# hpcaitech/Open-Sora

Hardware: AMD Instinct MI355X
Metric: latent_frames_per_sec (30-step rectified-flow sampling; denoise-step ms in ms_per_step) (higher is better)
Workload: dtype bf16; 1 GPU; MMDiT-XL (hidden 1152, 16x72, 9+19 blocks) denoise step, latent 16x64x64 (16x512x512 px), L=16896 tokens, CFG batch 3, 30-step Euler sampling; cfg_batch=3, parallelism=single GPU

## Files before the change

### open_sora_amd/csrc/gemm256x.hip

```cpp
#include "acc_quads.h"
#include "gemm_epilogue16.h"
#include "tile256.h"
#include "gemm256x_regs.inc"

namespace osk_gemm {
namespace {

struct GeoX {
  static constexpr int NB = OSKX_NB;
  template <int T>
  OSK_DEV void read(const osk_v4f* aq, float* v4) {
#pragma unroll
    for (int i = 0; i < 4; ++i) asm volatile("v_accvgpr_read_b32 %0, %1" : "=v"(v4[i]) : "a"(aq[T][i]));
  }
};

template <int NP>
struct GemmPack {
  GemmParams p[NP];
};

#ifdef OSK_GEMM_TILE_TIMING
__device__ unsigned long long osk_gemm_tile_ticks[4];
#define OSK_TT(i, t0) if (threadIdx.x == 0) atomicAdd(&osk_gemm_tile_ticks[i], __builtin_amdgcn_s_memtime() - (t0))
#else
#define OSK_TT(i, t0)
#endif


template <bool OUT_F32>
struct LinearWalk {
  template <int NP>
  OSK_DEV int col_tiles(const GemmPack<NP>& pk, int) { return (pk.p[0].N - pk.p[0].skip_len + 255) / 256; }
  template <int NP>
  OSK_DEV int phys_n0(const GemmPack<NP>& pk, int n0) { return n0 + (n0 >= pk.p[0].skip_from ? pk.p[0].skip_len : 0); }
  OSK_DEV int64_t a_row(const GemmParams& p, int m) { return osk_tile256::a_row_offset(p, m); }
  OSK_DEV int64_t w_row(const GemmParams& p, int n, bool) { return osk_tile256::w_row_offset(p, n); }
  OSK_DEV bool affine(const GemmParams& p, int m0, int n0) {
    return m0 + 256 <= p.M && n0 + 256 <= p.N && m0 / p.arpb == (m0 + 255) / p.arpb;
  }
  OSK_DEV int64_t a_origin(const GemmParams& p, int m0) { return osk_tile256::tile_window(m0, p.M, p.arpb, 0x7fffffff, p.abs_, p.ars).lo; }
  OSK_DEV int64_t w_origin(const GemmParams& p, int n0) { return osk_tile256::tile_window(n0, p.N, 0x7fffffff, 0x7fffffff, 0, p.wrs).lo; }
  OSK_DEV bool folded(const GemmParams& p, int n0w) { return p.bias != nullptr && n0w + OSKX_NB * 16 <= p.N; }
  OSK_DEV void epilogue(const osk_v4f* aq, const GemmParams& p, int m0w, int n0w, int l15, int q4, bool folded) {
    constexpr int WT = OSKX_NB * 16;
    const int b_first = m0w / p.crpb, b_last = (m0w + WT - 1) / p.crpb;
    const bool interior = m0w + WT <= p.M && n0w + WT <= p.N && b_first == b_last;
    epi16::epilogue_all<GeoX, OUT_F32>(aq, p, m0w, n0w, l15, q4, interior, folded);
  }
};

struct VtWalk {
  template <int NP>
  OSK_DEV int col_tiles(const GemmPack<NP>& pk, int i) { return (pk.p[i].N + 255) / 256; }
  template <int NP>
  OSK_DEV int phys_n0(const GemmPack<NP>&, int n0) { return n0; }
  OSK_DEV int64_t a_row(const GemmParams& p, int m) {
    m = m < p.M ? m : p.M - 1;
    return (int64_t)m * p.ars;
  }
  OSK_DEV int64_t w_row(const GemmParams& p, int n, bool permute) {
    n = n < p.N ? n : p.N - 1;
    const int wb = n / p.wrpb;
    int pos = n - wb * p.wrpb;
    if (permute) pos = vt_perm64(pos, p.vt);
    pos = pos < p.wvalid ? pos : p.wvalid - 1;
    return wb * p.wbs + (int64_t)pos * p.wrs;
  }
  OSK_DEV bool affine(const GemmParams& p, int m0, int n0) {
    const int wb = n0 / p.wrpb, pos0 = n0 - wb * p.wrpb;
    return m0 + 256 <= p.M && n0 + 256 <= p.N && pos0 + 256 <= p.wrpb && pos0 + 256 <= p.wvalid;
  }
  OSK_DEV int64_t a_origin(const GemmParams& p, int m0) { return osk_tile256::tile_window(m0, p.M, 0x7fffffff, 0x7fffffff, 0, p.ars).lo; }
  OSK_DEV int64_t w_origin(const GemmParams& p, int n0) { return osk_tile256::tile_window(n0, p.N, p.wrpb, p.wvalid, p.wbs, p.wrs).lo; }
  OSK_DEV bool folded(const GemmParams&, int) { return false; }
  OSK_DEV void epilogue(const osk_v4f* aq, const GemmParams& p, int m0w, int n0w, int l15, int q4, bool) {
    epi16::vt_all<GeoX>(aq, p, m0w, n0w, l15, q4);
  }
};

#define OSKW_OPERANDS                                                                                               \
  ::"v"(faA0), "v"(faW0), "v"(aoff[0]), "v"(aoff[1]), "v"(aoff[2]), "v"(aoff[3]), "v"(aoff[4]), "v"(aoff[5]),          \
      "v"(aoff[6]), "v"(aoff[7]), "v"(woff[0]), "v"(woff[1]), "v"(woff[2]), "v"(woff[3]), "v"(woff[4]), "v"(woff[5]),  \
      "v"(woff[6]), "v"(woff[7]), "v"(boff), "s"(abase), "s"(wbase), "s"(bbase), "s"(nk), "s"(adst), "s"(wdst),        \
      "s"(flags), "s"(abasen), "s"(wbasen), "v"(aoffp), "v"(woffp)

template <class Walk, int NP>
OSK_DEV void tile_walk(const GemmPack<NP>& pk) {
  constexpr int WT = OSKX_NB * 16;
  extern __shared__ __attribute__((aligned(16))) unsigned char smem[];
  const int tid = threadIdx.x;
  const int lane = tid & 63;
  const int wave = __builtin_amdgcn_readfirstlane(tid >> 6);
  const int wm = wave >> 1, wn = wave & 1;
  const int q4 = lane >> 4, l15 = lane & 15;

  const int nbn0 = Walk::col_tiles(pk, 0), nbn1 = Walk::col_tiles(pk, NP - 1);
  const int nt0 = ((pk.p[0].M + 255) / 256) * nbn0;
  const int ntiles = NP == 1 ? nt0 : nt0 + ((pk.p[NP - 1].M + 255) / 256) * nbn1;
  const int grp = pk.p[0].group > 0 ? pk.p[0].group : 1;
  auto tile_of = [&](int it, int& sel, int& m0, int& n0) {
    int tile = xcd_remap(it, ntiles);
    sel = (NP > 1 && tile >= nt0) ? 1 : 0;
    tile -= sel ? nt0 : 0;
    const osk_tile256::TileBlock t = osk_tile256::grouped_tile(tile, (pk.p[sel].M + 255) / 256, sel ? nbn1 : nbn0, grp);
    m0 = t.bm * 256;
    n0 = Walk::phys_n0(pk, t.bn * 256);
  };
  const unsigned lds_base = (unsigned)(uintptr_t)(__attribute__((address_space(3))) unsigned char*)smem;
  const unsigned sz0 = (unsigned)((q4 ^ ((l15 >> 1) & 7)) << 4);
  const unsigned faA0 = lds_base + (wm * WT + l15) * 128 + sz0;
  const unsigned faW0 = lds_base + OSKX_W_BASE + (wn * WT + l15) * 128 + sz0;
  const unsigned nk = rfl((unsigned)(pk.p[0].K / 64));
  const unsigned adst = rfl(lds_base + wave * 1024), wdst = rfl(lds_base + OSKX_W_BASE + wave * 1024);

  unsigned prefetched = 0;
  for (int it = blockIdx.x; it < ntiles; it += (int)gridDim.x) {
    const int itn = it + (int)gridDim.x;
#ifdef OSK_GEMM_TILE_TIMING
    const unsigned long long tt0 = __builtin_amdgcn_s_memtime();
#endif
    int sel, m0, n0, seln = 0, m0n = 0, n0n = 0;
    tile_of(it, sel, m0, n0);
    const GemmParams& p = pk.p[NP == 1 ? 0 : sel];
    bool has_next = itn < ntiles;
    const int64_t alo = Walk::a_origin(p, m0), wlo = Walk::w_origin(p, n0);
    int64_t alon = alo, wlon = wlo;
    if (has_next) {
      tile_of(itn, seln, m0n, n0n);
      has_next = seln == sel && Walk::affine(p, m0, n0) && Walk::affine(p, m0n, n0n);
      alon = Walk::a_origin(p, m0n);
      wlon = Walk::w_origin(p, n0n);
    }
    const uint64_t abase = rfl64((uint64_t)(uintptr_t)p.A + (uint64_t)(alo * 2)), wbase = rfl64((uint64_t)(uintptr_t)p.W + (uint64_t)(wlo * 2));
    const uint64_t abasen = rfl64((uint64_t)(uintptr_t)p.A + (uint64_t)(alon * 2)), wbasen = rfl64((uint64_t)(uintptr_t)p.W + (uint64_t)(wlon * 2));
    const uint64_t bbase = rfl64((uint64_t)(uintptr_t)p.bias);
    unsigned aoff[8], woff[8];
#pragma unroll
    for (int i = 0; i < 8; ++i) {
      const int r = osk_tile256::dma_row<4>(wave, lane, i);
      const int c = osk_tile256::dma_chunk(lane, r);
      aoff[i] = (unsigned)((Walk::a_row(p, m0 + r) - alo) * 2 + c * 16);
      woff[i] = (unsigned)((Walk::w_row(p, n0 + r, true) - wlo) * 2 + c * 16);
    }
    const int m0w = m0 + wm * WT, n0w = n0 + wn * WT;
    const bool folded = Walk::folded(p, n0w);
    const unsigned boff = (unsigned)((n0w + q4 * 4) * 4);
    const unsigned flags = rfl(prefetched | (has_next ? 2u : 0u) | (folded ? 4u : 0u));
    const unsigned aoffp = (unsigned)((Walk::a_row(p, m0 + wave * 64 + lane) - alo) * 2);
    const unsigned woffp = (unsigned)((Walk::w_row(p, n0 + wave * 64 + lane, false) - wlo) * 2);
    OSK_TT(0, tt0);
#ifdef OSK_GEMM_TILE_TIMING
    const unsigned long long tt1 = __builtin_amdgcn_s_memtime();
#endif
    asm volatile(
#include "gemm256x_body.inc"
        OSKW_OPERANDS : OSKX_CLOBBERS);
    static_assert(OSKX_ACC_QUADS == 64, "the generated loop's accumulator map: quad T = tile T, a0 .. a255");
    osk_v4f aq[64];
    asm volatile("" : OSK_AQ_OUT_0_64(aq));
    OSK_TT(1, tt1);
#ifdef OSK_GEMM_TILE_TIMING
    const unsigned long long tt2 = __builtin_amdgcn_s_memtime();
#endif
    Walk::epilogue(aq, p, m0w, n0w, l15, q4, folded);
    OSK_TT(2, tt2);
#ifdef OSK_GEMM_TILE_TIMING
    if (threadIdx.x == 0) atomicAdd(&osk_gemm_tile_ticks[3], 1ull);
#endif
    prefetched = has_next ? 1u : 0u;
  }
}

#undef OSKW_OPERANDS

template <bool OUT_F32, int NP>
__global__ void __launch_bounds__(256, 1) gemm256x_kernel(const GemmPack<NP> pk) {
  tile_walk<LinearWalk<OUT_F32>>(pk);
}

template <int NP>
__global__ void __launch_bounds__(256, 1) gemm256x_vt_kernel(const GemmPack<NP> pk) {
  static_assert(NP <= 2, "a run-time index into a wider pack makes hipcc copy the pack to scratch");
  tile_walk<VtWalk>(pk);
}

int tiles_of(const GemmParams& p) { return ((p.M + 255) / 256) * ((p.N - p.skip_len + 255) / 256); }

template <bool OUT_F32>
int launch_one(const GemmParams& p, hipStream_t st) {
  auto kernel = gemm256x_kernel<OUT_F32, 1>;
  OSK_ENSURE_MAX_SMEM(kernel, OSKX_SMEM);
  GemmPack<1> pk;
  pk.p[0] = p;
  hipLaunchKernelGGL(kernel, dim3(osk_tile256::persistent_grid(tiles_of(p))), dim3(256), OSKX_SMEM, st, pk);
  return (int)hipGetLastError();
}

}

#ifdef OSK_GEMM_TILE_TIMING
extern "C" int osk_gemm_tile_timing_read(unsigned long long* out4) {
  unsigned long long zero[4] = {0, 0, 0, 0};
  if (hipMemcpyFromSymbol(out4, HIP_SYMBOL(osk_gemm_tile_ticks), sizeof(zero)) != hipSuccess) return -1;
  return hipMemcpyToSymbol(HIP_SYMBOL(osk_gemm_tile_ticks), zero, sizeof(zero)) == hipSuccess ? 0 : -1;
}
#endif

int launch_gemm256x(const GemmParams& p, int out_f32, hipStream_t st) {
  return out_f32 ? launch_one<true>(p, st) : launch_one<false>(p, st);
}

int launch_gemm256x_pair(const GemmParams& p0, const GemmParams& p1, hipStream_t st) {
  auto kernel = gemm256x_kernel<false, 2>;
  OSK_ENSURE_MAX_SMEM(kernel, OSKX_SMEM);
  GemmPack<2> pk;
  pk.p[0] = p0;
  pk.p[1] = p1;
  hipLaunchKernelGGL(kernel, dim3(osk_tile256::persistent_grid(tiles_of(p0) + tiles_of(p1))), dim3(256), OSKX_SMEM, st, pk);
  return (int)hipGetLastError();
}

int launch_gemm256x_vt(const GemmParams* ps, int n, hipStream_t st) {
  if (n < 1 || n > 2) return OSK_EINVAL;
  auto kernel = gemm256x_vt_kernel<2>;
  OSK_ENSURE_MAX_SMEM(kernel, OSKX_SMEM);
  GemmPack<2> pk;
  int ntiles = 0;
  for (int i = 0; i < 2; ++i) {
    pk.p[i] = ps[i < n ? i : 0];
    if (i >= n) pk.p[i].M = 0;
    ntiles += tiles_of(pk.p[i]);
  }
  hipLaunchKernelGGL(kernel, dim3(osk_tile256::persistent_grid(ntiles)), dim3(256), OSKX_SMEM, st, pk);
  return (int)hipGetLastError();
}

}
```

### open_sora_amd/csrc/gemm256x_body.inc

```
"  s_mov_b64 s[40:41], %19\n"
"  s_mov_b64 s[42:43], %20\n"
"  s_mov_b64 s[54:55], %21\n"
"  s_mov_b32 s44, %22\n"
"  s_mov_b32 s45, %23\n"
"  s_mov_b32 s46, %24\n"
"  s_mov_b32 s52, %25\n"
"  s_mov_b32 s47, 0\n"
"  s_mov_b32 s48, 0\n"
"  v_xor_b32_e32 v224, 64, %0\n"
"  v_xor_b32_e32 v225, 64, %1\n"
"  s_bitcmp1_b32 s52, 0\n"
"  s_cbranch_scc1 .Lx256_have0_%=\n"
"  s_add_u32 m0, s45, 0\n"
"  s_nop 0\n"
"  global_load_lds_dwordx4 %2, s[40:41]\n"
"  s_add_u32 m0, s45, 4096\n"
"  s_nop 0\n"
"  global_load_lds_dwordx4 %3, s[40:41]\n"
"  s_add_u32 m0, s45, 8192\n"
"  s_nop 0\n"
"  global_load_lds_dwordx4 %4, s[40:41]\n"
"  s_add_u32 m0, s45, 12288\n"
"  s_nop 0\n"
"  global_load_lds_dwordx4 %5, s[40:41]\n"
"  s_add_u32 m0, s45, 16384\n"
"  s_nop 0\n"
"  global_load_lds_dwordx4 %6, s[40:41]\n"
"  s_add_u32 m0, s45, 20480\n"
"  s_nop 0\n"
"  global_load_lds_dwordx4 %7, s[40:41]\n"
"  s_add_u32 m0, s45, 24576\n"
"  s_nop 0\n"
"  global_load_lds_dwordx4 %8, s[40:41]\n"
"  s_add_u32 m0, s45, 28672\n"
"  s_nop 0\n"
"  global_load_lds_dwordx4 %9, s[40:41]\n"
"  s_add_u32 m0, s46, 0\n"
"  s_nop 0\n"
"  global_load_lds_dwordx4 %10, s[42:43]\n"
"  s_add_u32 m0, s46, 4096\n"
"  s_nop 0\n"
"  global_load_lds_dwordx4 %11, s[42:43]\n"
"  s_add_u32 m0, s46, 8192\n"
"  s_nop 0\n"
"  global_load_lds_dwordx4 %12, s[42:43]\n"
"  s_add_u32 m0, s46, 12288\n"
"  s_nop 0\n"
"  global_load_lds_dwordx4 %13, s[42:43]\n"
"  s_add_u32 m0, s46, 16384\n"
"  s_nop 0\n"
"  global_load_lds_dwordx4 %14, s[42:43]\n"
"  s_add_u32 m0, s46, 20480\n"
"  s_nop 0\n"
"  global_load_lds_dwordx4 %15, s[42:43]\n"
"  s_add_u32 m0, s46, 24576\n"
"  s_nop 0\n"
"  global_load_lds_dwordx4 %16, s[42:43]\n"
"  s_add_u32 m0, s46, 28672\n"
"  s_nop 0\n"
"  global_load_lds_dwordx4 %17, s[42:43]\n"
".Lx256_have0_%=:\n"
"  s_add_u32 s49, s48, 1\n"
"  s_cmp_lt_u32 s49, s44\n"
"  s_cselect_b32 s50, 128, 0\n"
"  s_cselect_b32 s48, s49, s48\n"
"  s_add_u32 s40, s40, s50\n"
"  s_addc_u32 s41, s41, 0\n"
"  s_add_u32 s42, s42, s50\n"
"  s_addc_u32 s43, s43, 0\n"
"  s_bitcmp1_b32 s52, 2\n"
"  s_cbranch_scc0 .Lx256_nobias_%=\n"
"  global_load_dwordx4 v[96:99], %18, s[54:55] offset:0\n"
"  global_load_dwordx4 v[100:103], %18, s[54:55] offset:64\n"
"  global_load_dwordx4 v[104:107], %18, s[54:55] offset:128\n"
"  global_load_dwordx4 v[108:111], %18, s[54:55] offset:192\n"
"  global_load_dwordx4 v[112:115], %18, s[54:55] offset:256\n"
"  global_load_dwordx4 v[116:119], %18, s[54:55] offset:320\n"
"  global_load_dwordx4 v[120:123], %18, s[54:55] offset:384\n"
"  global_load_dwordx4 v[124:127], %18, s[54:55] offset:448\n"
".Lx256_nobias_%=:\n"
"  s_waitcnt vmcnt(0)\n"
"  s_barrier\n"
"  s_bitcmp1_b32 s52, 0\n"
"  s_cbranch_scc1 .Lx256_have1_%=\n"
"  s_add_u32 m0, s45, 32768\n"
"  s_nop 0\n"
"  global_load_lds_dwordx4 %2, s[40:41]\n"
"  s_add_u32 m0, s45, 36864\n"
"  s_nop 0\n"
"  global_load_lds_dwordx4 %3, s[40:41]\n"
"  s_add_u32 m0, s45, 40960\n"
"  s_nop 0\n"
"  global_load_lds_dwordx4 %4, s[40:41]\n"
"  s_add_u32 m0, s45, 45056\n"
"  s_nop 0\n"
"  global_load_lds_dwordx4 %5, s[40:41]\n"
"  s_add_u32 m0, s45, 49152\n"
"  s_nop 0\n"
"  global_load_lds_dwordx4 %6, s[40:41]\n"
"  s_add_u32 m0, s45, 53248\n"
"  s_nop 0\n"
"  global_load_lds_dwordx4 %7, s[40:41]\n"
"  s_add_u32 m0, s45, 57344\n"
"  s_nop 0\n"
"  global_load_lds_dwordx4 %8, s[40:41]\n"
"  s_add_u32 m0, s45, 61440\n"
"  s_nop 0\n"
"  global_load_lds_dwordx4 %9, s[40:41]\n"
"  s_add_u32 m0, s46, 32768\n"
"  s_nop 0\n"
"  global_load_lds_dwordx4 %10, s[42:43]\n"
"  s_add_u32 m0, s46, 36864\n"
"  s_nop 0\n"
"  global_load_lds_dwordx4 %11, s[42:43]\n"
"  s_add_u32 m0, s46, 40960\n"
"  s_nop 0\n"
"  global_load_lds_dwordx4 %12, s[42:43]\n"
"  s_add_u32 m0, s46, 45056\n"
"  s_nop 0\n"
"  global_load_lds_dwordx4 %13, s[42:43]\n"
"  s_add_u32 m0, s46, 49152\n"
"  s_nop 0\n"
"  global_load_lds_dwordx4 %14, s[42:43]\n"
"  s_add_u32 m0, s46, 53248\n"
"  s_nop 0\n"
"  global_load_lds_dwordx4 %15, s[42:43]\n"
"  s_add_u32 m0, s46, 57344\n"
"  s_nop 0\n"
"  global_load_lds_dwordx4 %16, s[42:43]\n"
"  s_add_u32 m0, s46, 61440\n"
"  s_nop 0\n"
"  global_load_lds_dwordx4 %17, s[42:43]\n"
".Lx256_have1_%=:\n"
"  s_add_u32 s49, s48, 1\n"
"  s_cmp_lt_u32 s49, s44\n"
"  s_cselect_b32 s50, 128, 0\n"
"  s_cselect_b32 s48, s49, s48\n"
"  s_add_u32 s40, s40, s50\n"
"  s_addc_u32 s41, s41, 0\n"
"  s_add_u32 s42, s42, s50\n"
"  s_addc_u32 s43, s43, 0\n"
"  s_bitcmp1_b32 s52, 2\n"
"  s_cbranch_scc0 .Lx256_zero_%=\n"
"  v_accvgpr_write_b32 a0, v96\n"
"  v_accvgpr_write_b32 a1, v97\n"
"  v_accvgpr_write_b32 a2, v98\n"
"  v_accvgpr_write_b32 a3, v99\n"
"  v_accvgpr_write_b32 a4, v96\n"
"  v_accvgpr_write_b32 a5, v97\n"
"  v_accvgpr_write_b32 a6, v98\n"
"  v_accvgpr_write_b32 a7, v99\n"
"  v_accvgpr_write_b32 a8, v96\n"
"  v_accvgpr_write_b32 a9, v97\n"
"  v_accvgpr_write_b32 a10, v98\n"
"  v_accvgpr_write_b32 a11, v99\n"
"  v_accvgpr_write_b32 a12, v96\n"
"  v_accvgpr_write_b32 a13, v97\n"
"  v_accvgpr_write_b32 a14, v98\n"
"  v_accvgpr_write_b32 a15, v99\n"
"  v_accvgpr_write_b32 a16, v96\n"
"  v_accvgpr_write_b32 a17, v97\n"
"  v_accvgpr_write_b32 a18, v98\n"
"  v_accvgpr_write_b32 a19, v99\n"
"  v_accvgpr_write_b32 a20, v96\n"
"  v_accvgpr_write_b32 a21, v97\n"
"  v_accvgpr_write_b32 a22, v98\n"
"  v_accvgpr_write_b32 a23, v99\n"
"  v_accvgpr_write_b32 a24, v96\n"
"  v_accvgpr_write_b32 a25, v97\n"
"  v_accvgpr_write_b32 a26, v98\n"
"  v_accvgpr_write_b32 a27, v99\n"
"  v_accvgpr_write_b32 a28, v96\n"
"  v_accvgpr_write_b32 a29, v97\n"
"  v_accvgpr_write_b32 a30, v98\n"
"  v_accvgpr_write_b32 a31, v99\n"
"  v_accvgpr_write_b32 a32, v100\n"
"  v_accvgpr_write_b32 a33, v101\n"
"  v_accvgpr_write_b32 a34, v102\n"
"  v_accvgpr_write_b32 a35, v103\n"
"  v_accvgpr_write_b32 a36, v100\n"
"  v_accvgpr_write_b32 a37, v101\n"
"  v_accvgpr_write_b32 a38, v102\n"
"  v_accvgpr_write_b32 a39, v103\n"
"  v_accvgpr_write_b32 a40, v100\n"
"  v_accvgpr_write_b32 a41, v101\n"
"  v_accvgpr_write_b32 a42, v102\n"
"  v_accvgpr_write_b32 a43, v103\n"
"  v_accvgpr_write_b32 a44, v100\n"
"  v_accvgpr_write_b32 a45, v101\n"
"  v_accvgpr_write_b32 a46, v102\n"
"  v_accvgpr_write_b32 a47, v103\n"
"  v_accvgpr_write_b32 a48, v100\n"
"  v_accvgpr_write_b32 a49, v101\n"
"  v_accvgpr_write_b32 a50, v102\n"
"  v_accvgpr_write_b32 a51, v103\n"
"  v_accvgpr_write_b32 a52, v100\n"
"  v_accvgpr_write_b32 a53, v101\n"
"  v_accvgpr_write_b32 a54, v102\n"
"  v_accvgpr_write_b32 a55, v103\n"
"  v_accvgpr_write_b32 a56, v100\n"
"  v_accvgpr_write_b32 a57, v101\n"
"  v_accvgpr_write_b32 a58, v102\n"
"  v_accvgpr_write_b32 a59, v103\n"
"  v_accvgpr_write_b32 a60, v100\n"
"  v_accvgpr_write_b32 a61, v101\n"
"  v_accvgpr_write_b32 a62, v102\n"
"  v_accvgpr_write_b32 a63, v103\n"
"  v_accvgpr_write_b32 a64, v104\n"
"  v_accvgpr_write_b32 a65, v105\n"
"  v_accvgpr_write_b32 a66, v106\n"
"  v_accvgpr_write_b32 a67, v107\n"
"  v_accvgpr_write_b32 a68, v104\n"
"  v_accvgpr_write_b32 a69, v105\n"
"  v_accvgpr_write_b32 a70, v106\n"
"  v_accvgpr_write_b32 a71, v107\n"
"  v_accvgpr_write_b32 a72, v104\n"
"  v_accvgpr_write_b32 a73, v105\n"
"  v_accvgpr_write_b32 a74, v106\n"
"  v_accvgpr_write_b32 a75, v107\n"
"  v_accvgpr_write_b32 a76, v104\n"
"  v_accvgpr_write_b32 a77, v105\n"
"  v_accvgpr_write_b32 a78, v106\n"
"  v_accvgpr_write_b32 a79, v107\n"
"  v_accvgpr_write_b32 a80, v104\n"
"  v_accvgpr_write_b32 a81, v105\n"
"  v_accvgpr_write_b32 a82, v106\n"
"  v_accvgpr_write_b32 a83, v107\n"
"  v_accvgpr_write_b32 a84, v104\n"
"  v_accvgpr_write_b32 a85, v105\n"
"  v_accvgpr_write_b32 a86, v106\n"
"  v_accvgpr_write_b32 a87, v107\n"
"  v_accvgpr_write_b32 a88, v104\n"
"  v_accvgpr_write_b32 a89, v105\n"
"  v_accvgpr_write_b32 a90, v106\n"
"  v_accvgpr_write_b32 a91, v107\n"
"  v_accvgpr_write_b32 a92, v104\n"
"  v_accvgpr_write_b32 a93, v105\n"
"  v_accvgpr_write_b32 a94, v106\n"
"  v_accvgpr_write_b32 a95, v107\n"
"  v_accvgpr_write_b32 a96, v108\n"
"  v_accvgpr_write_b32 a97, v109\n"
"  v_accvgpr_write_b32 a98, v110\n"
"  v_accvgpr_write_b32 a99, v111\n"
"  v_accvgpr_write_b32 a100, v108\n"
"  v_accvgpr_write_b32 a101, v109\n"
"  v_accvgpr_write_b32 a102, v110\n"
"  v_accvgpr_write_b32 a103, v111\n"
"  v_accvgpr_write_b32 a104, v108\n"
"  v_accvgpr_write_b32 a105, v109\n"
"  v_accvgpr_write_b32 a106, v110\n"
"  v_accvgpr_write_b32 a107, v111\n"
"  v_accvgpr_write_b32 a108, v108\n"
"  v_accvgpr_write_b32 a109, v109\n"
"  v_accvgpr_write_b32 a110, v110\n"
"  v_accvgpr_write_b32 a111, v111\n"
"  v_accvgpr_write_b32 a112, v108\n"
"  v_accvgpr_write_b32 a113, v109\n"
"  v_accvgpr_write_b32 a114, v110\n"
"  v_accvgpr_write_b32 a115, v111\n"
"  v_accvgpr_write_b32 a116, v108\n"
"  v_accvgpr_write_b32 a117, v109\n"
"  v_accvgpr_write_b32 a118, v110\n"
"  v_accvgpr_write_b32 a119, v111\n"
"  v_accvgpr_write_b32 a120, v108\n"
"  v_accvgpr_write_b32 a121, v109\n"
"  v_accvgpr_write_b32 a122, v110\n"
"  v_accvgpr_write_b32 a123, v111\n"
"  v_accvgpr_write_b32 a124, v108\n"
"  v_accvgpr_write_b32 a125, v109\n"
"  v_accvgpr_write_b32 a126, v110\n"
"  v_accvgpr_write_b32 a127, v111\n"
"  v_accvgpr_write_b32 a128, v112\n"
"  v_accvgpr_write_b32 a129, v113\n"
"  v_accvgpr_write_b32 a130, v114\n"
"  v_accvgpr_write_b32 a131, v115\n"
"  v_accvgpr_write_b32 a132, v112\n"
"  v_accvgpr_write_b32 a133, v113\n"
"  v_accvgpr_write_b32 a134, v114\n"
"  v_accvgpr_write_b32 a135, v115\n"
"  v_accvgpr_write_b32 a136, v112\n"
"  v_accvgpr_write_b32 a137, v113\n"
"  v_accvgpr_write_b32 a138, v114\n"
"  v_accvgpr_write_b32 a139, v115\n"
"  v_accvgpr_write_b32 a140, v112\n"
"  v_accvgpr_write_b32 a141, v113\n"
"  v_accvgpr_write_b32 a142, v114\n"
"  v_accvgpr_write_b32 a143, v115\n"
"  v_accvgpr_write_b32 a144, v112\n"
"  v_accvgpr_write_b32 a145, v113\n"
"  v_accvgpr_write_b32 a146, v114\n"
"  v_accvgpr_write_b32 a147, v115\n"
"  v_accvgpr_write_b32 a148, v112\n"
"  v_accvgpr_write_b32 a149, v113\n"
"  v_accvgpr_write_b32 a150, v114\n"
"  v_accvgpr_write_b32 a151, v115\n"
"  v_accvgpr_write_b32 a152, v112\n"
"  v_accvgpr_write_b32 a153, v113\n"
"  v_accvgpr_write_b32 a154, v114\n"
"  v_accvgpr_write_b32 a155, v115\n"
"  v_accvgpr_write_b32 a156, v112\n"
"  v_accvgpr_write_b32 a157, v113\n"
"  v_accvgpr_write_b32 a158, v114\n"
"  v_accvgpr_write_b32 a159, v115\n"
"  v_accvgpr_write_b32 a160, v116\n"
"  v_accvgpr_write_b32 a161, v117\n"
"  v_accvgpr_write_b32 a162, v118\n"
"  v_accvgpr_write_b32 a163, v119\n"
"  v_accvgpr_write_b32 a164, v116\n"
"  v_accvgpr_write_b32 a165, v117\n"
"  v_accvgpr_write_b32 a166, v118\n"
"  v_accvgpr_write_b32 a167, v119\n"
"  v_accvgpr_write_b32 a168, v116\n"
"  v_accvgpr_write_b32 a169, v117\n"
"  v_accvgpr_write_b32 a170, v118\n"
"  v_accvgpr_write_b32 a171, v119\n"
"  v_accvgpr_write_b32 a172, v116\n"
"  v_accvgpr_write_b32 a173, v117\n"
"  v_accvgpr_write_b32 a174, v118\n"
"  v_accvgpr_write_b32 a175, v119\n"
"  v_accvgpr_write_b32 a176, v116\n"
"  v_accvgpr_write_b32 a177, v117\n"
"  v_accvgpr_write_b32 a178, v118\n"
"  v_accvgpr_write_b32 a179, v119\n"
"  v_accvgpr_write_b32 a180, v116\n"
"  v_accvgpr_write_b32 a181, v117\n"
"  v_accvgpr_write_b32 a182, v118\n"
"  v_accvgpr_write_b32 a183, v119\n"
"  v_accvgpr_write_b32 a184, v116\n"
"  v_accvgpr_write_b32 a185, v117\n"
"  v_accvgpr_write_b32 a186, v118\n"
"  v_accvgpr_write_b32 a187, v119\n"
"  v_accvgpr_write_b32 a188, v116\n"
"  v_accvgpr_write_b32 a189, v117\n"
"  v_accvgpr_write_b32 a190, v118\n"
"  v_accvgpr_write_b32 a191, v119\n"
"  v_accvgpr_write_b32 a192, v120\n"
"  v_accvgpr_write_b32 a193, v121\n"
"  v_accvgpr_write_b32 a194, v122\n"
"  v_accvgpr_write_b32 a195, v123\n"
"  v_accvgpr_write_b32 a196, v120\n"
"  v_accvgpr_write_b32 a197, v121\n"
"  v_accvgpr_write_b32 a198, v122\n"
"  v_accvgpr_write_b32 a199, v123\n"
"  v_accvgpr_write_b32 a200, v120\n"
"  v_accvgpr_write_b32 a201, v121\n"
"  v_accvgpr_write_b32 a202, v122\n"
"  v_accvgpr_write_b32 a203, v123\n"
"  v_accvgpr_write_b32 a204, v120\n"
"  v_accvgpr_write_b32 a205, v121\n"
"  v_accvgpr_write_b32 a206, v122\n"
"  v_accvgpr_write_b32 a207, v123\n"
"  v_accvgpr_write_b32 a208, v120\n"
"  v_accvgpr_write_b32 a209, v121\n"
"  v_accvgpr_write_b32 a210, v122\n"
"  v_accvgpr_write_b32 a211, v123\n"
"  v_accvgpr_write_b32 a212, v120\n"
"  v_accvgpr_write_b32 a213, v121\n"
"  v_accvgpr_write_b32 a214, v122\n"
"  v_accvgpr_write_b32 a215, v123\n"
"  v_accvgpr_write_b32 a216, v120\n"
"  v_accvgpr_write_b32 a217, v121\n"
"  v_accvgpr_write_b32 a218, v122\n"
"  v_accvgpr_write_b32 a219, v123\n"
"  v_accvgpr_write_b32 a220, v120\n"
"  v_accvgpr_write_b32 a221, v121\n"
"  v_accvgpr_write_b32 a222, v122\n"
"  v_accvgpr_write_b32 a223, v123\n"
"  v_accvgpr_write_b32 a224, v124\n"
"  v_accvgpr_write_b32 a225, v125\n"
"  v_accvgpr_write_b32 a226, v126\n"
"  v_accvgpr_write_b32 a227, v127\n"
"  v_accvgpr_write_b32 a228, v124\n"
"  v_accvgpr_write_b32 a229, v125\n"
"  v_accvgpr_write_b32 a230, v126\n"
"  v_accvgpr_write_b32 a231, v127\n"
"  v_accvgpr_write_b32 a232, v124\n"
"  v_accvgpr_write_b32 a233, v125\n"
"  v_accvgpr_write_b32 a234, v126\n"
"  v_accvgpr_write_b32 a235, v127\n"
"  v_accvgpr_write_b32 a236, v124\n"
"  v_accvgpr_write_b32 a237, v125\n"
"  v_accvgpr_write_b32 a238, v126\n"
// ... 936 lines not shown
```

Baseline: 4.282 latent frames/s.

## Permute weight rows so GEMM epilogue stores eight contiguous columns per lane

Adds a column-permuted variant of the 256x256 GEMM. Weight rows are loaded in permuted order so each lane's two accumulator quads map to eight contiguous output columns. A new epilogue writes 16-byte bf16 stores (or paired float4 stores), and the bias prefetch in the asm loop is adjusted to match. The goal is wider, fewer global stores and residual loads in the epilogue, at the cost of more code paths and index remapping on the DMA offsets.

```diff
diff --git a/open_sora_amd/csrc/gemm256x.hip b/open_sora_amd/csrc/gemm256x.hip
--- a/open_sora_amd/csrc/gemm256x.hip
+++ b/open_sora_amd/csrc/gemm256x.hip
@@ -1,5 +1,6 @@
 #include "acc_quads.h"
 #include "gemm_epilogue16.h"
+#include "gemm_epilogue16p.h"
 #include "tile256.h"
 #include "gemm256x_regs.inc"
 
@@ -42,11 +43,14 @@
   OSK_DEV int64_t a_origin(const GemmParams& p, int m0) { return osk_tile256::tile_window(m0, p.M, p.arpb, 0x7fffffff, p.abs_, p.ars).lo; }
   OSK_DEV int64_t w_origin(const GemmParams& p, int n0) { return osk_tile256::tile_window(n0, p.N, 0x7fffffff, 0x7fffffff, 0, p.wrs).lo; }
   OSK_DEV bool folded(const GemmParams& p, int n0w) { return p.bias != nullptr && n0w + OSKX_NB * 16 <= p.N; }
+  OSK_DEV bool permuted(const GemmParams& p) { return epi16p::use_perm<OUT_F32>(p); }
   OSK_DEV void epilogue(const osk_v4f* aq, const GemmParams& p, int m0w, int n0w, int l15, int q4, bool folded) {
     constexpr int WT = OSKX_NB * 16;
     const int b_first = m0w / p.crpb, b_last = (m0w + WT - 1) / p.crpb;
     const bool interior = m0w + WT <= p.M && n0w + WT <= p.N && b_first == b_last;
-    epi16::epilogue_all<GeoX, OUT_F32>(aq, p, m0w, n0w, l15, q4, interior, folded);
+    if (permuted(p)) epi16p::epilogue_all<GeoX, OUT_F32>(aq, p, m0w, n0w, l15, q4, interior, folded);
+    else if constexpr (!epi16p::ALL_CLASSES) epi16::epilogue_all<GeoX, OUT_F32>(aq, p, m0w, n0w, l15, q4, interior, folded);
+    else if constexpr (!OUT_F32) epi16::geglu_all<GeoX>(aq, p, m0w, n0w, l15, q4, interior, folded);
   }
 };
 
@@ -74,6 +78,7 @@
   OSK_DEV int64_t a_origin(const GemmParams& p, int m0) { return osk_tile256::tile_window(m0, p.M, 0x7fffffff, 0x7fffffff, 0, p.ars).lo; }
   OSK_DEV int64_t w_origin(const GemmParams& p, int n0) { return osk_tile256::tile_window(n0, p.N, p.wrpb, p.wvalid, p.wbs, p.wrs).lo; }
   OSK_DEV bool folded(const GemmParams&, int) { return false; }
+  OSK_DEV bool permuted(const GemmParams&) { return false; }
   OSK_DEV void epilogue(const osk_v4f* aq, const GemmParams& p, int m0w, int n0w, int l15, int q4, bool) {
     epi16::vt_all<GeoX>(aq, p, m0w, n0w, l15, q4);
   }
@@ -135,18 +140,20 @@
     const uint64_t abase = rfl64((uint64_t)(uintptr_t)p.A + (uint64_t)(alo * 2)), wbase = rfl64((uint64_t)(uintptr_t)p.W + (uint64_t)(wlo * 2));
     const uint64_t abasen = rfl64((uint64_t)(uintptr_t)p.A + (uint64_t)(alon * 2)), wbasen = rfl64((uint64_t)(uintptr_t)p.W + (uint64_t)(wlon * 2));
     const uint64_t bbase = rfl64((uint64_t)(uintptr_t)p.bias);
+    const bool perm = Walk::permuted(p);
     unsigned aoff[8], woff[8];
 #pragma unroll
     for (int i = 0; i < 8; ++i) {
       const int r = osk_tile256::dma_row<4>(wave, lane, i);
       const int c = osk_tile256::dma_chunk(lane, r);
+      const int rw = perm ? (r & 128) | epi16p::perm_col(r & 127) : r;
       aoff[i] = (unsigned)((Walk::a_row(p, m0 + r) - alo) * 2 + c * 16);
-      woff[i] = (unsigned)((Walk::w_row(p, n0 + r, true) - wlo) * 2 + c * 16);
+      woff[i] = (unsigned)((Walk::w_row(p, n0 + rw, true) - wlo) * 2 + c * 16);
     }
     const int m0w = m0 + wm * WT, n0w = n0 + wn * WT;
     const bool folded = Walk::folded(p, n0w);
-    const unsigned boff = (unsigned)((n0w + q4 * 4) * 4);
-    const unsigned flags = rfl(prefetched | (has_next ? 2u : 0u) | (folded ? 4u : 0u));
+    const unsigned boff = (unsigned)((n0w + q4 * (perm ? 8 : 4)) * 4);
+    const unsigned flags = rfl(prefetched | (has_next ? 2u : 0u) | (folded ? 4u : 0u) | (perm ? 8u : 0u));
     const unsigned aoffp = (unsigned)((Walk::a_row(p, m0 + wave * 64 + lane) - alo) * 2);
     const unsigned woffp = (unsigned)((Walk::w_row(p, n0 + wave * 64 + lane, false) - wlo) * 2);
     OSK_TT(0, tt0);
diff --git a/open_sora_amd/csrc/gemm256x_body.inc b/open_sora_amd/csrc/gemm256x_body.inc
--- a/open_sora_amd/csrc/gemm256x_body.inc
+++ b/open_sora_amd/csrc/gemm256x_body.inc
@@ -70,6 +70,8 @@
 "  s_addc_u32 s43, s43, 0\n"
 "  s_bitcmp1_b32 s52, 2\n"
 "  s_cbranch_scc0 .Lx256_nobias_%=\n"
+"  s_bitcmp1_b32 s52, 3\n"
+"  s_cbranch_scc1 .Lx256_permbias_%=\n"
 "  global_load_dwordx4 v[96:99], %18, s[54:55] offset:0\n"
 "  global_load_dwordx4 v[100:103], %18, s[54:55] offset:64\n"
 "  global_load_dwordx4 v[104:107], %18, s[54:55] offset:128\n"
@@ -78,6 +80,16 @@
 "  global_load_dwordx4 v[116:119], %18, s[54:55] offset:320\n"
 "  global_load_dwordx4 v[120:123], %18, s[54:55] offset:384\n"
 "  global_load_dwordx4 v[124:127], %18, s[54:55] offset:448\n"
+"  s_branch .Lx256_nobias_%=\n"
+".Lx256_permbias_%=:\n"
+"  global_load_dwordx4 v[96:99], %18, s[54:55] offset:0\n"
+"  global_load_dwordx4 v[100:103], %18, s[54:55] offset:16\n"
+"  global_load_dwordx4 v[104:107], %18, s[54:55] offset:128\n"
+"  global_load_dwordx4 v[108:111], %18, s[54:55] offset:144\n"
+"  global_load_dwordx4 v[112:115], %18, s[54:55] offset:256\n"
+"  global_load_dwordx4 v[116:119], %18, s[54:55] offset:272\n"
+"  global_load_dwordx4 v[120:123], %18, s[54:55] offset:384\n"
+"  global_load_dwordx4 v[124:127], %18, s[54:55] offset:400\n"
 ".Lx256_nobias_%=:\n"
 "  s_waitcnt vmcnt(0)\n"
 "  s_barrier\n"
diff --git a/open_sora_amd/csrc/gemm_epilogue16p.h b/open_sora_amd/csrc/gemm_epilogue16p.h
--- /dev/null
+++ b/open_sora_amd/csrc/gemm_epilogue16p.h
@@ -0,0 +1,166 @@
+#pragma once
+#include "gemm_epilogue16.h"
+
+namespace osk_gemm {
+namespace epi16p {
+
+using epi::GELU_ALL;
+using epi::GELU_MIXED;
+using epi::GELU_NONE;
+
+static __host__ __device__ __forceinline__ int perm_col(int rho) {
+  return (rho & ~31) | (((rho >> 2) & 3) << 3) | (((rho >> 4) & 1) << 2) | (rho & 3);
+}
+template <int J>
+OSK_DEV int tile_col(int q4) { return 32 * (J >> 1) + 4 * (J & 1) + 8 * q4; }
+
+#ifndef OSK_GEMM_PERM_CLASSES
+#define OSK_GEMM_PERM_CLASSES 15
+#endif
+constexpr bool ALL_CLASSES = (OSK_GEMM_PERM_CLASSES & 15) == 15;
+template <bool OUT_F32>
+OSK_DEV bool use_perm(const GemmParams& p) {
+  constexpr int mask = OSK_GEMM_PERM_CLASSES;
+  if (p.geglu || p.vt) return false;
+  if constexpr (OUT_F32) return (mask & 8) != 0;
+  if (p.gate) return (mask & 4) != 0;
+  return p.gelu_from < p.N ? (mask & 2) != 0 : (mask & 1) != 0;
+}
+
+template <int GELU>
+OSK_DEV void activate(const GemmParams& p, int n, float* v8) {
+  if constexpr (GELU == GELU_ALL) {
+#pragma unroll
+    for (int i = 0; i < 8; ++i) v8[i] = gelu_tanh(v8[i]);
+  } else if constexpr (GELU == GELU_MIXED) {
+#pragma unroll
+    for (int i = 0; i < 8; ++i) {
+      const float g = gelu_tanh(v8[i]);
+      v8[i] = n + i >= p.gelu_from ? g : v8[i];
+    }
+  }
+}
+
+template <bool RES16>
+OSK_DEV uint4 load_res(const unsigned short* r) {
+  if constexpr (RES16) return *reinterpret_cast<const uint4*>(r);
+  const uint2 lo = *reinterpret_cast<const uint2*>(r), hi = *reinterpret_cast<const uint2*>(r + 4);
+  return make_uint4(lo.x, lo.y, hi.x, hi.y);
+}
+
+template <class Geo, bool OUT_F32, bool GATE, int GELU, int I, int A>
+OSK_DEV void pair_store(const osk_v4f* aq, const GemmParams& p, int64_t roff, int n0w, int q4, const float4* gq, const uint4& rv) {
+  constexpr int NB = Geo::NB;
+  const int n = n0w + 32 * A + 8 * q4;
+  float v[8];
+  Geo::template read<(2 * A) * NB + I>(aq, v);
+  Geo::template read<(2 * A + 1) * NB + I>(aq, v + 4);
+  activate<GELU>(p, n, v);
+  if constexpr (GATE) {
+    const float4 g0 = gq[2 * A], g1 = gq[2 * A + 1];
+    v[0] = bf16_lo(rv.x) + g0.x * v[0];
+    v[1] = bf16_hi(rv.x) + g0.y * v[1];
+    v[2] = bf16_lo(rv.y) + g0.z * v[2];
+    v[3] = bf16_hi(rv.y) + g0.w * v[3];
+    v[4] = bf16_lo(rv.z) + g1.x * v[4];
+    v[5] = bf16_hi(rv.z) + g1.y * v[5];
+    v[6] = bf16_lo(rv.w) + g1.z * v[6];
+    v[7] = bf16_hi(rv.w) + g1.w * v[7];
+  }
+  if constexpr (OUT_F32) {
+    float* c = reinterpret_cast<float*>(p.C) + roff + n;
+    *reinterpret_cast<float4*>(c) = make_float4(v[0], v[1], v[2], v[3]);
+    *reinterpret_cast<float4*>(c + 4) = make_float4(v[4], v[5], v[6], v[7]);
+  } else {
+    *reinterpret_cast<uint4*>(reinterpret_cast<unsigned short*>(p.C) + roff + n) =
+        make_uint4(pack_bf16x2(v[0], v[1]), pack_bf16x2(v[2], v[3]), pack_bf16x2(v[4], v[5]), pack_bf16x2(v[6], v[7]));
+  }
+}
+
+template <class Geo, bool OUT_F32, bool GATE, int GELU, bool RES16, int I, int... As>
+OSK_DEV void row_pair(const osk_v4f* aq, const GemmParams& p, int64_t row0, int64_t step, int n0w, int q4, const float4* gq,
+                      std::integer_sequence<int, As...>) {
+  constexpr int NP = Geo::NB / 2;
+  const int64_t rowoff[2] = {row0 + I * step, row0 + (I + 1) * step};
+  uint4 r0[NP], r1[NP];
+#pragma unroll
+  for (int a = 0; a < NP; ++a) {
+    r0[a] = r1[a] = make_uint4(0, 0, 0, 0);
+    if constexpr (GATE) {
+      r0[a] = load_res<RES16>(p.res + rowoff[0] + n0w + 32 * a + 8 * q4);
+      r1[a] = load_res<RES16>(p.res + rowoff[1] + n0w + 32 * a + 8 * q4);
+    }
+  }
+  (pair_store<Geo, OUT_F32, GATE, GELU, I, As>(aq, p, rowoff[0], n0w, q4, gq, r0[As]), ...);
+  (pair_store<Geo, OUT_F32, GATE, GELU, I + 1, As>(aq, p, rowoff[1], n0w, q4, gq, r1[As]), ...);
+}
+
+template <class Geo, bool OUT_F32, bool GATE, int GELU, bool RES16, int... Is>
+OSK_DEV void tile_interior(const osk_v4f* aq, const GemmParams& p, int64_t row0, int64_t step, int n0w, int q4, const float4* gq,
+                           std::integer_sequence<int, Is...>) {
+  (row_pair<Geo, OUT_F32, GATE, GELU, RES16, 2 * Is>(aq, p, row0, step, n0w, q4, gq, std::make_integer_sequence<int, Geo::NB / 2>{}), ...);
+}
+
+template <class Geo, bool OUT_F32, bool GATE, bool RES16>
+OSK_DEV void cols_interior(const osk_v4f* aq, const GemmParams& p, int64_t row0, int64_t step, int m0w, int n0w, int q4) {
+  constexpr int NB = Geo::NB;
+  constexpr auto seq = std::make_integer_sequence<int, NB / 2>{};
+  float4 gq[NB];
+#pragma unroll
+  for (int j = 0; j < NB; ++j) {
+    gq[j] = make_float4(0.f, 0.f, 0.f, 0.f);
+    if constexpr (GATE) gq[j] = *reinterpret_cast<const float4*>(p.gate + (m0w / p.crpb) * p.gbs + n0w + 32 * (j >> 1) + 8 * q4 + 4 * (j & 1));
+  }
+  if (n0w + NB * 16 <= p.gelu_from) tile_interior<Geo, OUT_F32, GATE, GELU_NONE, RES16>(aq, p, row0, step, n0w, q4, gq, seq);
+  else if (n0w >= p.gelu_from) tile_interior<Geo, OUT_F32, GATE, GELU_ALL, RES16>(aq, p, row0, step, n0w, q4, gq, seq);
+  else tile_interior<Geo, OUT_F32, GATE, GELU_MIXED, RES16>(aq, p, row0, step, n0w, q4, gq, seq);
+}
+
+template <class Geo, bool OUT_F32, int T>
+OSK_DEV void tile_edge(const osk_v4f* aq, const GemmParams& p, int m0w, int n0w, int l15, int q4, bool folded) {
+  constexpr int NB = Geo::NB;
+  constexpr int J = T / NB, I = T % NB;
+  float acc[4];
+  Geo::template read<T>(aq, acc);
+  const int m = m0w + I * 16 + l15;
+  if (m >= p.M) return;
+  const int b = m / p.crpb, l = m - b * p.crpb;
+  const int64_t roff = b * p.cbs + (int64_t)l * p.crs;
+  const float* grow = p.gate ? p.gate + b * p.gbs : nullptr;
+  const int n = n0w + tile_col<J>(q4);
+  for (int j = 0; j < 4 && n + j < p.N; ++j) {
+    float t = acc[j];
+    if (!folded && p.bias) t += p.bias[n + j];
+    if (n + j >= p.gelu_from) t = gelu_tanh(t);
+    if (grow) t = bf16_bits_to_f32(p.res[roff + n + j]) + grow[n + j] * t;
+    if constexpr (OUT_F32) reinterpret_cast<float*>(p.C)[roff + n + j] = t;
+    else reinterpret_cast<unsigned short*>(p.C)[roff + n + j] = f32_to_bf16_bits(t);
+  }
+}
+
+template <class Geo, bool OUT_F32, int... Ts>
+OSK_DEV void tiles_edge(const osk_v4f* aq, const GemmParams& p, int m0w, int n0w, int l15, int q4, bool folded, std::integer_sequence<int, Ts...>) {
+  (tile_edge<Geo, OUT_F32, Ts>(aq, p, m0w, n0w, l15, q4, folded), ...);
+}
+
+template <class Geo, bool OUT_F32>
+OSK_DEV void epilogue_all(const osk_v4f* aq, const GemmParams& p, int m0w, int n0w, int l15, int q4, bool interior, bool folded) {
+  constexpr int NB = Geo::NB;
+  if (m0w >= p.M || n0w >= p.N) return;
+  const bool wide = OUT_F32 || (((((uintptr_t)p.C) & 15) == 0) && ((p.crs & 7) == 0) && ((p.cbs & 7) == 0));
+  if (!interior || !wide || (p.bias && !folded)) {
+    tiles_edge<Geo, OUT_F32>(aq, p, m0w, n0w, l15, q4, folded, std::make_integer_sequence<int, NB * NB>{});
+    return;
+  }
+  const int b = m0w / p.crpb, l0 = m0w - b * p.crpb + l15;
+  const int64_t row0 = b * p.cbs + (int64_t)l0 * p.crs, step = 16 * p.crs;
+  if (p.gate) {
+    if ((((uintptr_t)p.res) & 15) == 0) cols_interior<Geo, OUT_F32, true, true>(aq, p, row0, step, m0w, n0w, q4);
+    else cols_interior<Geo, OUT_F32, true, false>(aq, p, row0, step, m0w, n0w, q4);
+  } else {
+    cols_interior<Geo, OUT_F32, false, true>(aq, p, row0, step, m0w, n0w, q4);
+  }
+}
+
+}
+}
```

Result: no change. 4.312 latent frames/s (median of 6 runs) (+0.7%).
